# CEED/Laghos

Measured on AMD Instinct MI355X. Metric: Mdofs×steps/s on 3D Sedov -pa (Q3/Q2), higher is better.
Workload: dtype f64; 1 GPU; 3D Sedov -p 1 -m cube01_hex -rs 4 -ok 3 -ot 2 -pa (32^3 elements, E0/2^dim = 0.125); transport=none (one rank), elements=32768, h1_dofs=2738019, l2_dofs=884736, quad_points_per_element=216, rk_stages_executed=1300, ode=RK4, parallelism=elements1x1x1, zones_per_gpu=32x32x32

## Files before the change

include/laghos_hip.h:

```cpp
#ifndef LAGHOS_HIP_H
#define LAGHOS_HIP_H

#ifdef __cplusplus
extern "C" {
#endif

#define LGH_OK 0
#define LGH_ERR_ARG 1
#define LGH_ERR_UNSUPPORTED 2
#define LGH_ERR_HIP 3
#define LGH_ERR_COMM 4

#define LGH_SPACE_H1 0
#define LGH_SPACE_L2 1

typedef struct lgh_ctx lgh_ctx;

typedef struct lgh_config
{
   int dim, NE;
   int D1D, Q1D, L1D;
   int N;
   const int *h1_map;
   const double *B_h1;
// ... 38 lines not shown
int lgh_force_mult(lgh_ctx *ctx, const double *x_l2, double *y_h1);
int lgh_force_mult_transpose(lgh_ctx *ctx, const double *v_h1, double *y_l2);

int lgh_mass_set_essential_tdofs(lgh_ctx *ctx, int comp);
int lgh_mass_eliminate_rhs(lgh_ctx *ctx, double *b);
int lgh_mass_mult(lgh_ctx *ctx, int space, const double *x, double *y);
int lgh_mass_mult_full(lgh_ctx *ctx, int space, const double *x, double *y);

int lgh_cg_solve(lgh_ctx *ctx, int space, const double *b, double *x, double rel_tol,
                 int max_iter, int *iters);
int lgh_l2_mass_solve_local(lgh_ctx *ctx, const double *b, double *x);

int lgh_qupdate(lgh_ctx *ctx, const double *S);
int lgh_qupdate_set_tiny_grad(lgh_ctx *ctx, double tiny_grad);
int lgh_set_fused_forces(lgh_ctx *ctx, int on);
int lgh_qupdate_store_stress(lgh_ctx *ctx, int on);
int lgh_qupdate_stores_stress(lgh_ctx *ctx, int *on);
int lgh_qupdate_form(lgh_ctx *ctx, int *form);
int lgh_reset_quadrature_data(lgh_ctx *ctx);
int lgh_fused_force_mult(lgh_ctx *ctx, double *y_h1);
int lgh_fused_force_mult_transpose(lgh_ctx *ctx, double *y_l2);
int lgh_quadrature_generation(lgh_ctx *ctx, unsigned long *gen, int *f1_valid, int *ftv_valid);
int lgh_get_fused_forces(lgh_ctx *ctx, int *f1, int *ftv);

int lgh_solve_velocity(lgh_ctx *ctx, const double *S, double *dS_dt, const double *one_l2,
                       double *rhs_h1, double *work_B, double rel_tol, int max_iter,
                       int *h1_iters);
int lgh_solve_energy(lgh_ctx *ctx, const double *S, const double *v_h1, double *dS_dt,
                     double *e_rhs, const double *e_source, double rel_tol, int max_iter,
                     int *l2_iters);
// ... 117 lines not shown
```

laghos_amd/_lib.py:

```python
import ctypes
import os

_HERE = os.path.dirname(os.path.abspath(__file__))
LIB_PATH = os.path.join(_HERE, "liblaghos_hip.so")

c_dp = ctypes.c_void_p
c_int_p = ctypes.POINTER(ctypes.c_int)
c_dbl_p = ctypes.POINTER(ctypes.c_double)


class LghConfig(ctypes.Structure):
    _fields_ = [
        ("dim", ctypes.c_int), ("NE", ctypes.c_int),
        ("D1D", ctypes.c_int), ("Q1D", ctypes.c_int), ("L1D", ctypes.c_int),
        ("N", ctypes.c_int),
        ("h1_map", c_int_p),
        ("B_h1", c_dbl_p), ("G_h1", c_dbl_p), ("B_l2", c_dbl_p),
        ("weights", c_dbl_p), ("gamma", c_dbl_p),
        ("ess_count", ctypes.c_int * 3),
        ("ess", c_int_p * 3),
        ("owner", c_dbl_p),
        ("use_viscosity", ctypes.c_int), ("use_vorticity", ctypes.c_int),
        ("cfl", ctypes.c_double),
        ("order_v", ctypes.c_int),
# ... 22 lines not shown
    "lgh_mass_diag": (_P, [_P]),
    "lgh_set_h0": (_I, [_P, _D]),
    "lgh_get_h0": (_I, [_P, c_dbl_p]),
    "lgh_set_dt_est": (_I, [_P, _D]),
    "lgh_get_dt_est": (_I, [_P, c_dbl_p]),
    "lgh_setup_rho0detj0": (_I, [_P, _P, _P, _P, c_dbl_p]),
    "lgh_force_mult": (_I, [_P, _P, _P]),
    "lgh_force_mult_transpose": (_I, [_P, _P, _P]),
    "lgh_mass_set_essential_tdofs": (_I, [_P, _I]),
    "lgh_mass_eliminate_rhs": (_I, [_P, _P]),
    "lgh_mass_mult": (_I, [_P, _I, _P, _P]),
    "lgh_mass_mult_full": (_I, [_P, _I, _P, _P]),
    "lgh_cg_solve": (_I, [_P, _I, _P, _P, _D, _I, c_int_p]),
    "lgh_l2_mass_solve_local": (_I, [_P, _P, _P]),
    "lgh_qupdate": (_I, [_P, _P]),
    "lgh_solve_velocity": (_I, [_P, _P, _P, _P, _P, _P, _D, _I, c_int_p]),
    "lgh_solve_energy": (_I, [_P, _P, _P, _P, _P, _P, _D, _I, c_int_p]),
    "lgh_solve_energy_begin": (_I, [_P, _P, _P, _P, _P, _P, _D, _I]),
    "lgh_tg_source_2d": (_I, [_P, _P, _P]),
    "lgh_set_velocity_source": (_I, [_P, _P]),
    "lgh_solve_energy_end": (_I, [_P, c_int_p]),
    "lgh_vec_set": (_I, [_P, _P, _D, _L]),
    "lgh_vec_copy": (_I, [_P, _P, _P, _L]),
    "lgh_vec_axpby": (_I, [_P, _P, _D, _P, _D, _P, _L]),
    "lgh_vec_axpby_pair": (_I, [_P, _P, _D, _P, _D, _P, _D, _P, _D, _P, _L]),
    "lgh_vec_dot": (_I, [_P, _P, _P, _L, c_dbl_p]),
    "lgh_vec_fingerprint": (_I, [_P, _P, _L, ctypes.c_ulonglong, ctypes.POINTER(ctypes.c_ulonglong)]),
    "lgh_vec_fingerprint_shape": (_I, [_P, _P, _L, ctypes.POINTER(ctypes.c_long)]),
    "lgh_fingerprint_host": (_I, [_P, _L, ctypes.c_ulonglong, ctypes.POINTER(ctypes.c_ulonglong)]),
    "lgh_internal_energy": (_I, [_P, _P, c_dbl_p]),
# ... 98 lines not shown
```

laghos_amd/context.py:

```python
import ctypes

import numpy as np
import torch

from . import _lib
from ._lib import LghConfig, check


def _np_i32(a):
    return np.ascontiguousarray(a, dtype=np.int32)


def _np_f64(a):
    return np.ascontiguousarray(a, dtype=np.float64)


def _ptr(t):
    assert t.is_cuda and t.dtype == torch.float64 and t.is_contiguous()
    return ctypes.c_void_p(t.data_ptr())


def _dbl(a):
    assert isinstance(a, np.ndarray) and a.dtype == np.float64 and a.flags.c_contiguous
    return a.ctypes.data_as(_lib.c_dbl_p)
# ... 205 lines not shown
    def mass_mult(self, space, x, y, full=False):
        fn = self.lib.lgh_mass_mult_full if full else self.lib.lgh_mass_mult
        check(fn(self.h, space, _ptr(x), _ptr(y)))

    def cg_solve(self, space, b, x, rel_tol, max_iter):
        it = ctypes.c_int(0)
        check(self.lib.lgh_cg_solve(self.h, space, _ptr(b), _ptr(x), rel_tol, max_iter, ctypes.byref(it)))
        return it.value

    def l2_mass_solve_local(self, b, x):
        check(self.lib.lgh_l2_mass_solve_local(self.h, _ptr(b), _ptr(x)))

    def qupdate(self, S):
        check(self.lib.lgh_qupdate(self.h, _ptr(S)))

    def qupdate_set_tiny_grad(self, v):
        check(self.lib.lgh_qupdate_set_tiny_grad(self.h, float(v)))

    def table_symmetry(self):
        a, b = ctypes.c_int(-1), ctypes.c_int(-1)
        check(self.lib.lgh_table_symmetry(self.h, ctypes.byref(a), ctypes.byref(b)))
        return a.value, b.value

    def k1_form(self):
        f = ctypes.c_int(-2)
        check(self.lib.lgh_k1_form(self.h, ctypes.byref(f)))
        return {0: "column", 2: "plane", 4: "slab", 5: "kron"}.get(f.value)

    def mesh_order(self):
        o = (ctypes.c_long * 8)()
# ... 273 lines not shown
```

laghos_amd/csrc/lgh_api.hip:

```cpp
#include <cstdarg>
#include <cstdlib>
#include <cmath>
#include <algorithm>
#include <limits>

#include "lgh_common.hpp"

#include <chrono>
#include <dlfcn.h>

namespace lgh
{

static thread_local char g_err[512] = "";
void set_error(const char *fmt, ...)
{
   va_list ap;
   va_start(ap, fmt);
   vsnprintf(g_err, sizeof(g_err), fmt, ap);
   va_end(ap);
}

__global__ void __launch_bounds__(256) vec_set_k(double *y, double a, long n)
{
// ... 489 lines not shown
   LGH_TRY(dev_alloc_zero(&c->Jac0inv_e, (size_t)cfg->NE * dim * dim));
   LGH_TRY(dev_alloc_zero(&c->rho0DetJ0w, nq));
   LGH_TRY(dev_alloc_zero(&c->massD, nq + 2048));
   LGH_TRY(dev_alloc_zero(&c->diagV, (size_t)c->N));
   LGH_TRY(dev_alloc_zero(&c->dinvV, (size_t)c->N));
   LGH_TRY(dev_alloc_zero(&c->dt_est_dev, (size_t)kDtSlotStride * (1 + kDtSlots)));
   {
      const char *env = getenv("LGH_FUSED_FTV");
      if (!(env && env[0] == '0'))
      {
         LGH_TRY(dev_alloc_zero(&c->erhs_q, (size_t)c->L2V));
         LGH_TRY(dev_alloc_zero(&c->v_snap, (size_t)c->H1V));
      }
      LGH_TRY(dev_alloc_zero(&c->dev_flags, (size_t)8));
      c->mass_rank1 = -1;
      env = getenv("LGH_FUSED_F1");
      if (c->dim == 3 && !(env && env[0] == '0')) { LGH_TRY(dev_alloc_zero(&c->force_e_q, nmap * dim + (size_t)dim * c->ND)); }
   }
   const size_t ne_nd = nmap * dim;
   LGH_TRY(dev_alloc_zero(&c->XE, std::max<size_t>(ne_nd, (size_t)c->L2V)));
   LGH_TRY(dev_alloc_zero(&c->YE, ne_nd + (size_t)dim * c->ND));
   const size_t nv = std::max<size_t>((size_t)c->N, (size_t)c->L2V);
   LGH_TRY(dev_alloc_zero(&c->cg_r, nv));
   LGH_TRY(dev_alloc_zero(&c->cg_z, nv));
   LGH_TRY(dev_alloc_zero(&c->cg_d0, nv));
   LGH_TRY(dev_alloc_zero(&c->cg_d1, nv));
   LGH_TRY(dev_alloc_zero(&c->cg_y, nv));
   c->part_stride = (int)std::max<size_t>(std::max<size_t>((size_t)c->NE, (nv + 255) / 256), 2048) + (int)kShards;
   LGH_TRY(dev_alloc_zero(&c->partials, 4 * (size_t)c->part_stride));
   LGH_TRY(dev_alloc_zero(&c->tickets, 4 * (size_t)kTicketSlot));
// ... 269 lines not shown
   if (c->dim == 1) { return cg_1d(c, space, b, x, rel_tol, max_iter, iters, false); }
   return cg_solve(c, space, b, x, rel_tol, max_iter, iters, false);
}

int lgh_l2_mass_solve_local(lgh_ctx *c, const double *b, double *x)
{
   LGH_CHECK_ARG(c && b && x);
   if (c->dim != 1)
   {
      set_error("lgh_l2_mass_solve_local: the zone-local energy solve belongs to the 1D (full-assembly) path; 2D/3D run the energy CG");
      return LGH_ERR_UNSUPPORTED;
   }
   return l2_solve_local_1d(c, b, x);
}

int lgh_qupdate(lgh_ctx *c, const double *S)
{
   LGH_CHECK_ARG(c && S);
   RoctxRange range("QUpdate-UpdateQuadratureData");
   timer_start(c);
   kt_begin(c, LGH_KERNEL_QUPDATE);
   int rc = (c->dim == 1) ? qupdate_1d(c, S) : qupdate(c, S);
   kt_end(c, LGH_KERNEL_QUPDATE);
   timer_stop(c, 3);
   c->timers.c[2] += c->NE;
   return rc;
}

__global__ void __launch_bounds__(256) not_all_ones_k(const double *x, const long n, int *flag)
{
   const long i = (long)blockIdx.x * blockDim.x + threadIdx.x;
   if (i < n && x[i] != 1.0) { *flag = 1; }
}
static bool is_the_one_vector(lgh_ctx *c, const double *one_l2)
{
   if (!one_l2) { return true; }
   int *flag = c->dev_flags + 1;
   if (hipMemsetAsync(flag, 0, sizeof(int), c->stream) != hipSuccess) { return false; }
   hipLaunchKernelGGL(not_all_ones_k, dim3(ceil_div(c->L2V, 256)), dim3(256), 0, c->stream, one_l2, (long)c->L2V, flag);
   int h = 1;
   if (hipMemcpyAsync(&h, flag, sizeof(int), hipMemcpyDeviceToHost, c->stream) != hipSuccess) { return false; }
// ... 163 lines not shown
   if (i < n) { y[i] = x[i]; }
}
__global__ void __launch_bounds__(256) copy_unless_k(double *__restrict__ y, const double *__restrict__ x, const long n, const int *__restrict__ flag)
{
   if (*flag != 0) { return; }
   const long i = (long)blockIdx.x * blockDim.x + threadIdx.x;
   if (i < n) { y[i] = x[i]; }
}
static int energy_rhs(lgh_ctx *c, const double *v_h1, double *e_rhs)
{
   RoctxRange range("SolveEnergy-ForcePA");
   if (c->erhs_q && c->fused_ftv_valid)
   {
      int *flag = c->dev_flags + (c->on_stream2 ? 2 : 0);
      LGH_HIP_CHECK(hipMemsetAsync(flag, 0, sizeof(int), c->stream));
      hipLaunchKernelGGL(vec_differs_k, dim3(grid_for((c->H1V + 1) / 2)), dim3(256), 0, c->stream, v_h1, c->v_snap, (long)c->H1V, flag);
      LGH_HIP_CHECK(hipGetLastError());
      if (c->stress_current)
      {
         const int rc = force_mult_t_L(c, c->stressJinvT, v_h1, e_rhs, flag);
         if (rc) { return rc; }
         hipLaunchKernelGGL(copy_unless_k, dim3(ceil_div(c->L2V, 256)), dim3(256), 0, c->stream, e_rhs, c->erhs_q, (long)c->L2V, flag);
      }
      else
      {
         hipLaunchKernelGGL(erhs_take_or_poison_k, dim3(ceil_div(c->L2V, 256)), dim3(256), 0, c->stream, e_rhs, c->erhs_q, (long)c->L2V, flag, c->dev_flags + 4);
      }
      LGH_HIP_CHECK(hipGetLastError());
      return LGH_OK;
   }
   return lgh_force_mult_transpose(c, v_h1, e_rhs);
// ... 420 lines not shown
```

laghos_amd/csrc/lgh_common.hpp:

```cpp
#pragma once
#include <hip/hip_runtime.h>

#include <cstdint>
#include <cstdio>
#include <cstring>
#include <string>
#include <vector>

#include "../../include/laghos_hip.h"

namespace lgh
{

void set_error(const char *fmt, ...);

#define LGH_HIP_CHECK(expr)                                                              \
   do                                                                                    \
   {                                                                                     \
      hipError_t e_ = (expr);                                                            \
      if (e_ != hipSuccess)                                                              \
      {                                                                                  \
         lgh::set_error("HIP error %s at %s:%d: %s", hipGetErrorName(e_), __FILE__,      \
                        __LINE__, #expr);                                                \
         return LGH_ERR_HIP;                                                             \
// ... 88 lines not shown
   int ess_count[3];
   double *owner;
   int cur_ess;

   double *stressJinvT, *Jac0inv, *rho0DetJ0w, *massD, *diagV, *dinvV;
   double *Jac0inv_soa;
   double *Jac0inv_e;
   int jac0_compact;
   double *massS, *ones_ne;
   double *M1h = nullptr, *M1l = nullptr;
   double *w1d = nullptr;
   int mass_rank1;
   double *dt_est_dev;
   double *erhs_q;
   double *v_snap;
   double *force_e_q;
   int fused_ftv_valid, fused_f1_valid;
   unsigned long qgen;
   int *dev_flags;
   double *ones_l2;
   int stress_store;
   int stress_current;
   int fused_forces_off;
   double *XE;
   double *YE;
   double *cg_r, *cg_z, *cg_d0, *cg_d1, *cg_y;
   double *partials;
   int part_stride;
   unsigned int *tickets;
   lgh::CgScalars *cgs;
// ... 274 lines not shown
struct LockstepWords { const long long *own; const long long *peers; int n_peers, before; };
bool l2_lockstep_possible(lgh_ctx *c);
int cg_l2_begin_lockstep(lgh_ctx *c, const double *b, double *x, double rel_tol, int max_iter);
int l2_lockstep_limit(lgh_ctx *c);
int l2_lockstep_apply(lgh_ctx *c, int it, const LockstepWords &prev, double *den_mirror);
int l2_lockstep_update(lgh_ctx *c, int it, const double *den_src, long long *word_out);
int l2_lockstep_fold(lgh_ctx *c, int it, const LockstepWords &last);
int cg_l2_end_lockstep(lgh_ctx *c, int *iters);
int comm_ranks_before(const lgh_ctx *c);
bool vcg_lockstep_ready(const lgh_ctx *c);
int cg_l2_begin(lgh_ctx *c, const double *b, double *x, double rel_tol, int max_iter);
int cg_l2_end(lgh_ctx *c, int *iters);
void cg_l2_free(lgh_ctx *c);
int cg_solve(lgh_ctx *c, int space, const double *b, double *x, double rel_tol, int max_iter,
             int *iters, bool x_is_zero);
int qupdate(lgh_ctx *c, const double *S);
int setup_rho0detj0(lgh_ctx *c, const double *x0, const double *rho0_l2, const double *rho0_q,
                    double *volume);
int interp_energy(lgh_ctx *c, int which, const double *vec, double *result);
int tg_source_2d(lgh_ctx *c, const double *S, double *out);
int test_eig(lgh_ctx *c, int dim, int n, const double *A, double *lambda, double *vec);
int test_singular(lgh_ctx *c, int dim, int n, const double *A, double *sv);
int test_sqrt(lgh_ctx *c, int n, const double *x, double *y);
int vec_set(lgh_ctx *c, double *y, double a, long n);
int vec_axpby(lgh_ctx *c, double *z, double a, const double *x, double b, const double *y, long n);
int vec_axpby_pair(lgh_ctx *c, double *z1, double a1, const double *x1, double b1, double *z2, double a2, const double *x2, double b2,
                   const double *y, long n);
int vec_neg_inplace(lgh_ctx *c, double *y, long n);
int vec_zero_list(lgh_ctx *c, double *y, const int *list, int n);
int vec_dot(lgh_ctx *c, const double *x, const double *y, const double *w, long n, double *dev_out);
struct HaloNodeAlias { const int *nodes, *sh_node; };
// ... 70 lines not shown
```

laghos_amd/csrc/lgh_qupdate.hip:

```cpp
#include "lgh_qpoint.hpp"
#include "lgh_qrows.hpp"

namespace lgh
{

int qupdate_form(lgh_ctx *c);
int qupdate(lgh_ctx *c, const double *S)
{
   QArgs a = q_base(c);
   a.x = S;
   a.v = S + c->H1V;
   a.e = S + 2 * (size_t)c->H1V;
   a.result = c->dt_est_dev;
   a.Jac0inv_e = (c->jac0_compact == 1) ? c->Jac0inv_e : nullptr;
   const bool keep = !c->stress_store && a.erhs_q && a.force_e && c->v_snap;
   if (keep) { a.stressJinvT = nullptr; }
   const int form = qupdate_form(c);
   const int rc = (form == 1) ? launch_qrows(c, a) : launch_q<QMODE_UPDATE>(c, a);
   c->qgen++;
   c->stress_current = (rc == LGH_OK && !keep) ? 1 : 0;
   c->fused_ftv_valid = (rc == LGH_OK && a.erhs_q && c->v_snap) ? 1 : 0;
   c->fused_f1_valid = (rc == LGH_OK && a.force_e) ? 1 : 0;
   if (c->fused_ftv_valid)
   {
      LGH_HIP_CHECK(hipMemcpyAsync(c->v_snap, S + c->H1V, sizeof(double) * (size_t)c->H1V, hipMemcpyDeviceToDevice, c->stream));
   }
   return rc;
}

int qupdate_form(lgh_ctx *c)
{
   const char *fenv = getenv("LGH_Q_FORM");
   return (qrows_available(c) && !(fenv && fenv[0] == '0')) ? 1 : 0;
}

int interp_energy(lgh_ctx *c, int which, const double *vec, double *result)
{
   QArgs a = q_base(c);
   a.result = c->scal;
   int rc;
// ... 130 lines not shown
```

laghos_amd/csrc/lgh_vcg.hip:

```cpp
#include "lgh_vcg.hpp"

namespace lgh
{
typedef unsigned v4u_ __attribute__((ext_vector_type(4)));


template <int D, int Q, int NEB>
__global__ void __launch_bounds__(Q *Q *NEB, (Q >= 8) ? 1 : 2)
vcg_apply_3d(const VcgArgs a, const int nbatch)
{
   constexpr int NQ = Q * Q * Q, ND = D * D * D;
   constexpr int SX = (ND > D * Q * Q) ? ND : D * Q * Q;
   constexpr int SA = D * D * Q;
   constexpr int SAE = (SA > D * Q * D) ? SA : D * Q * D;
   constexpr int OFF_A = kVC * SX, OFF_IN = OFF_A + kVC * SAE;
   constexpr int PER = OFF_IN + kVC * ND + 1;
   constexpr int NT = Q * Q * NEB;
   constexpr int GPT = (NEB * ND + NT - 1) / NT;
   __shared__ double smem[NEB * PER];
   __shared__ double red[48];

   if (a.s->all_done) { return; }
   const int tid = threadIdx.x;
   const int tx = tid % Q, ty = (tid / Q) % Q, eb = tid / (Q * Q);
// ... 986 lines not shown
         VcgScalars *s = a.s;
         int all = 1;
         vcg_reset_scalars(a, s);
         for (int c = 0; c < kVC; c++)
         {
            s->rz[c] = s->rz_prev[c] = total[c];
            s->iters[c] = 0;
            s->r0[c] = fmax(total[c] * s->rel_tol2, 0.0);
            s->done[c] = (total[c] < 0.0 || total[c] <= s->r0[c]) ? 1 : 0;
            all = all && s->done[c];
         }
         s->first = 1;
         s->all_done = all;
      }
   }
}
__global__ void __launch_bounds__(256)
vcg_ellf_k(const int *__restrict__ ell, unsigned *__restrict__ ellf, const size_t n_have, const size_t n_all, const int ND, const int NE)
{
   const size_t i = (size_t)blockIdx.x * blockDim.x + threadIdx.x;
   if (i >= n_all) { return; }
   const int p = (i < n_have) ? ell[i] : -1;
   const int e = p / ND;
   ellf[i] = 8u * (unsigned)(p < 0 ? kVC * ND * NE : kVC * ND * e + (p - e * ND));
}
__global__ void __launch_bounds__(256)
vcg_mapb_k(const int *__restrict__ map, unsigned *__restrict__ mapb, const size_t n)
{
   const size_t i = (size_t)blockIdx.x * blockDim.x + threadIdx.x;
   if (i < n) { mapb[i] = 8u * (unsigned)map[i]; }
// ... 431 lines not shown
            }
            all = all && s->done[k];
         }
         if (!a.multi) { s->all_done = all; }
         if (a.pack_rz)
         {
            for (int k = 0; k < a.hp.n_nbr; k++)
            {
               for (int e = 0; e < kVC; e++) { a.hp.sbuf[(size_t)a.hp.base[k] + e] = s->rz[e]; }
            }
         }
      }
   }
}
__global__ void __launch_bounds__(256)
vcg_xfix_k(const VcgArgs a)
{
   const int n = blockIdx.x * blockDim.x + threadIdx.x;
   if (n >= a.N) { return; }
   for (int k = 0; k < kVC; k++)
   {
      if ((a.s->nupd[k] & 1) == 0) { continue; }
      const size_t i = (size_t)k * a.N + n;
      a.x[i] = fma(a.s->alpha_last[k], a.d[i], a.x[i]);
   }
}

__global__ void __launch_bounds__(256)
vcg_xout_k(const VcgArgs a, double *__restrict__ X)
{
   const int n = blockIdx.x * blockDim.x + threadIdx.x;
   if (n >= a.N) { return; }
   const int nc = a.ncaller[n];
   for (int k = 0; k < kVC; k++)
   {
      const size_t i = (size_t)k * a.N + n;
      double xv = a.x[i];
      if (a.s->nupd[k] & 1) { xv = fma(a.s->alpha_last[k], a.d[i], xv); }
      X[(size_t)k * a.N + nc] = xv;
   }
}

__global__ void __launch_bounds__(256)
vcg_gather_k(const VcgArgs a)
{
   const int n = blockIdx.x * blockDim.x + threadIdx.x;
   if (n >= a.N) { return; }
   for (int c = 0; c < kVC; c++)
   {
      if (a.s->done[c]) { continue; }
      const double *yc = a.YE + (size_t)c * a.ye_stride;
      double s = 0.0;
// ... 179 lines not shown
   if (c->multi) { comm_shared_nodes(c, &hmask, &sh_node, &n_shared); }
   hipLaunchKernelGGL(vcg_essbits_k, dim3((unsigned)((c->N + 255) / 256)), dim3(256), 0, nullptr, c->essmask[0], c->essmask[1],
                      c->essmask[2], hmask, c->multi ? c->owner : nullptr, *out, c->N);
   LGH_HIP_CHECK(hipGetLastError());
   return LGH_OK;
}


struct VcgAux
{
   double *ye = nullptr;
   unsigned *ellz = nullptr;
   uint8_t *essbits = nullptr;
   int *nstart = nullptr;
   unsigned *ellf = nullptr;
   unsigned *mapb = nullptr;
   int map_xrows = 0;
   long long *limbs = nullptr;
   long long *rzl = nullptr;
   int grid2 = 0;
   int rz_words_all = -1;
   int rz_words_key = -1;
   int ls_all = 0;
   int ls_ready = 0;
   unsigned *settab = nullptr;
   int *ellm = nullptr;
   int degm = 0;
   unsigned *ellzm = nullptr;
   int *nstartm = nullptr;
   const MeshOrder *ord = nullptr;
// ... 18 lines not shown
   return LGH_OK;
}
void vcg_free(lgh_ctx *c)
{
   VcgAux *x = (VcgAux *)c->vcg_aux;
   if (!x) { return; }
   (void)hipFree(x->settab);
   (void)hipFree(x->ellm);
   (void)hipFree(x->ellzm);
   (void)hipFree(x->nstartm);
   (void)hipFree(x->ye);
   (void)hipFree(x->ellz);
   (void)hipFree(x->essbits);
   (void)hipFree(x->nstart);
   (void)hipFree(x->ellf);
   (void)hipFree(x->mapb);
   (void)hipFree(x->limbs);
   (void)hipFree(x->rzl);
   (void)hipFree(x->o_map);
   (void)hipFree(x->o_ell);
   (void)hipFree(x->o_ellc);
   for (int k = 0; k < kVC; k++) { (void)hipFree(x->o_ess[k]); }
   (void)hipFree(x->o_dinv);
   (void)hipFree(x->o_Se);
   (void)hipFree(x->o_massD);
   (void)hipFree(x->o_x);
   (void)hipFree(x->o_owner);
   (void)hipFree(x->o_hmask);
   (void)hipFree(x->o_nodes);
   (void)hipFree(x->o_shnode);
// ... 276 lines not shown
         {
            uint8_t *tmp = nullptr;
            LGH_HIP_CHECK(hipMalloc((void **)&tmp, (size_t)c->N));
            LGH_HIP_CHECK(hipStreamSynchronize(nullptr));
            rc = order_gather_bytes(c, x->essbits, tmp);
            if (rc) { (void)hipFree(tmp); return rc; }
            LGH_HIP_CHECK(hipStreamSynchronize(c->stream));
            (void)hipFree(x->essbits);
            x->essbits = tmp;
         }
         rc = partition_nodes_by_cost(c, x->grid2, &x->nstart, x->ord ? &x->o_valence : nullptr);
         if (rc) { return rc; }
         if ((size_t)kVC * (c->NE + 1) * c->ND * 8 < 0xffffffffull)
         {
            const size_t ell_n = (size_t)8 * c->N;
            LGH_HIP_CHECK(hipMalloc((void **)&x->ellf, ell_n * sizeof(unsigned)));
            hipLaunchKernelGGL(vcg_ellf_k, dim3((unsigned)((ell_n + 255) / 256)), dim3(256), 0, nullptr, x->o_ellc ? x->o_ellc : c->t_ell, x->ellf,
                               (size_t)c->t_deg * c->N, ell_n, c->ND, c->NE);
            LGH_HIP_CHECK(hipGetLastError());
         }
      }
      if (vcg_k1_form(c) == 4)
      {
         const size_t nm = (size_t)c->NE * c->ND;
         LGH_HIP_CHECK(hipMalloc((void **)&x->mapb, nm * sizeof(unsigned)));
         hipLaunchKernelGGL(vcg_mapb_k, dim3((unsigned)((nm + 255) / 256)), dim3(256), 0, nullptr, v_map, x->mapb, nm);
         LGH_HIP_CHECK(hipGetLastError());
         int *flag = (int *)c->scal, h = 1;
         LGH_HIP_CHECK(hipMemset(flag, 0, sizeof(int)));
         hipLaunchKernelGGL(vcg_map_xrows_k, dim3((unsigned)((nm / c->D1D + 255) / 256)), dim3(256), 0, nullptr, v_map, nm / c->D1D, c->D1D, flag);
         LGH_HIP_CHECK(hipMemcpy(&h, flag, sizeof(int), hipMemcpyDeviceToHost));
         x->map_xrows = (h == 0) ? 1 : 0;
         LGH_HIP_CHECK(hipMalloc((void **)&x->limbs, (2 * kLimbWords + 8 * 16 + 32 * 4096) * sizeof(long long)));
// ... 241 lines not shown
int vcg_solve(lgh_ctx *c, double *B, double *X, double rel_tol, int max_iter, int iters[3], const double *force_E)
{
   if (!vcg_supported(c)) { return LGH_ERR_UNSUPPORTED; }
   VcgPlan plan;
   int rc = vcg_prepare(c, B, X, rel_tol, plan, true);
   if (rc) { return rc; }
   VcgArgs &a = plan.a;
   VcgAux *aux = plan.aux;
   const bool k2p = plan.k2p;
   const bool multi = c->multi != 0;
   const size_t N = (size_t)c->N;
   VcgScalars *ds = (VcgScalars *)c->vcg_s;
   const int nb = ceil_div((long)N, 256);
   const HaloNodeAlias *alias = (aux->ord && aux->o_alias.nodes) ? &aux->o_alias : nullptr;

   a.partials = c->vcg_partials;
   a.ticket = c->vcg_tickets;
   if (force_E)
   {
      if (multi || c->t_deg > 8) { set_error("vcg_solve: fused init is single-rank, degree <= 8"); return LGH_ERR_ARG; }
      if (aux->ellf && aux->essbits)
      {
         hipLaunchKernelGGL(vcg_init_force_z_k, dim3(nb), dim3(256), 0, c->stream, a, force_E, 8u * (unsigned)c->ND, aux->ellf, B);
      }
      else { hipLaunchKernelGGL(vcg_init_force_k<8>, dim3(nb), dim3(256), 0, c->stream, a, force_E, c->ND, B, aux->o_ellc ? aux->o_ellc : c->t_ell, c->t_deg); }
   }
   else
   {
      if (aux->ord) { LGH_HIP_CHECK(hipMemsetAsync(a.x, 0, kVC * N * sizeof(double), c->stream)); }
      hipLaunchKernelGGL(vcg_init_k, dim3(nb), dim3(256), 0, c->stream, a);
   }
   LGH_HIP_CHECK(hipGetLastError());
   if (multi)
   {
      rc = allreduce_dev(c, ds->rz, kVC, 0);
      if (rc) { return rc; }
// ... 25 lines not shown
   if (ls_side) { rc = hand_over(c->ev_fork, false); if (rc) { return rc; } }
   int chunk = c->vcg_last > 0 ? c->vcg_last : 8;
   bool first_look = true;
   while (true)
   {
      if (!first_look || max_iter <= 0)
      {
         VcgScalars *hs_dev = (VcgScalars *)(c->host_pinned_dev + 32);
         unsigned long long *tok_dev = (unsigned long long *)(c->host_pinned_dev + 80);
         volatile unsigned long long *tok = (volatile unsigned long long *)(c->host_pinned + 80);
         const unsigned long long token = ++c->look_token;
         bool copied = false;
         if (!energy_polled) { rc = energy_overlap_poll(c); energy_polled = true; if (rc) { return rc; } }
         if (multi && !a.rzl && it > 0) { hipLaunchKernelGGL(vcg_update_finish_k, dim3(1), dim3(1), 0, c->stream, ds, it, hs_dev, tok_dev, token); copied = true; }
         if (a.rzl && it > 0) { hipLaunchKernelGGL(vcg_rz_finish_k, dim3(1), dim3(1), 0, c->stream, ds, a.rzl, it, a.rzl_peers, a.n_rz_peers, hs_dev, tok_dev, token); copied = true; }
         if (copied)
         {
            rc = host_wait_token(c, tok, token);
            if (rc) { return rc; }
         }
         else
         {
            LGH_HIP_CHECK(hipMemcpyAsync(hs, ds, sizeof(VcgScalars), hipMemcpyDeviceToHost, c->stream));
            LGH_HIP_CHECK(hipStreamSynchronize(c->stream));
         }
         if (hs->all_done || it >= max_iter) { break; }
         chunk = (++looks <= 2) ? 2 : std::min(64, 2 * chunk);
      }
      first_look = false;
      const int upto = std::min(max_iter, it + chunk);
// ... 77 lines not shown
               {
                  rc = side([&] { return l2_lockstep_fold(c, it, ls_words(it)); });
                  if (rc) { return rc; }
               }
            }
            else if (multi)
            {
               rc = allreduce_dev(c, ds->rz, kVC, 0, a.pack_rz != 0 && mixed && k2p);
               if (rc) { return rc; }
            }
         }
         LGH_HIP_CHECK(hipGetLastError());
      }
   }
   if (ls_side) { rc = hand_over(c->ev_join, true); if (rc) { return rc; } }
   if (aux->ord)
   {
      hipLaunchKernelGGL(vcg_xout_k, dim3(nb), dim3(256), 0, c->stream, a, X);
      LGH_HIP_CHECK(hipGetLastError());
   }
   else if (k2p && ((hs->nupd[0] | hs->nupd[1] | hs->nupd[2]) & 1))
   {
      hipLaunchKernelGGL(vcg_xfix_k, dim3(nb), dim3(256), 0, c->stream, a);
      LGH_HIP_CHECK(hipGetLastError());
   }
   if (trace_dev)
   {
      std::vector<unsigned long long> h(kTraceRec * 4096);
      (void)hipMemcpy(h.data(), trace_dev, h.size() * 8, hipMemcpyDeviceToHost);
      FILE *f = fopen(trace_path, "w");
      if (f)
      {
         for (int i = 0; i < 4096; i++)
         {
            if (h[(size_t)kTraceRec * i] == 0) { continue; }
            fprintf(f, "%d", i);
            for (int k = 0; k < kTraceRec; k++) { fprintf(f, " %llu", h[(size_t)kTraceRec * i + k]); }
            fprintf(f, "\n");
// ... 423 lines not shown
```

laghos_amd/host/laghos_solver.cpp:

```cpp
#include "laghos_solver.hpp"

#include <cmath>
#include <cstdlib>
#include <cstring>
#include <iomanip>
#include <iostream>
#include <limits>

namespace laghos
{
namespace hydrodynamics
{

void AbortWithLghError(const char *where)
{
   std::fprintf(stderr, "%s failed: %s\n", where, lgh_last_error());
   std::abort();
}

LagrangianHydroOperator::LagrangianHydroOperator(const Discretization &d, const std::vector<double> &S0,
                                                 const std::vector<double> &rho0_l2,
                                                 const std::vector<double> &gamma,
                                                 const std::vector<double> &rho0_q, double cfl,
                                                 double cgt, int cgiter, int device, const char *nccl_id)
// ... 82 lines not shown
   {
      std::vector<double> acc((size_t)H1Vsize, 0.0);
      for (long i = H1Vsize / dim; i < 2 * (H1Vsize / dim); i++) { acc[i] = -1.0; }
      accel_src.FromHost(acc);
      LGH_VERIFY(lgh_set_velocity_source(ctx, accel_src.Read()));
   }
   B.SetSize(d.N);
   LGH_VERIFY(lgh_sync(ctx));
}

LagrangianHydroOperator::~LagrangianHydroOperator() { lgh_destroy(ctx); }

void LagrangianHydroOperator::Mult(const Vector &S, Vector &dS_dt) const
{
   UpdateMesh(S);
   LGH_VERIFY(lgh_vec_copy(ctx, dS_dt.Write(), S.Read() + H1Vsize, H1Vsize));
   UpdateQuadratureData(S);
   if (source_type == 1) { LGH_VERIFY(lgh_tg_source_2d(ctx, S.Read(), e_source.Write())); }
   LGH_VERIFY(lgh_solve_energy_begin(ctx, S.Read(), S.Read() + H1Vsize, dS_dt.Write(), e_rhs.Write(),
                                     source_type == 1 ? e_source.Read() : nullptr, cg_rel_tol, cg_max_iter));
   SolveVelocity(S, dS_dt);
   int it = 0;
   LGH_VERIFY(lgh_solve_energy_end(ctx, &it));
   qdata_is_current = false;
}

void LagrangianHydroOperator::SolveVelocity(const Vector &S, Vector &dS_dt) const
{
   UpdateQuadratureData(S);
   int it = 0;
   LGH_VERIFY(lgh_solve_velocity(ctx, S.Read(), dS_dt.Write(), nullptr, rhs.Write(), B.Write(),
                                 cg_rel_tol, cg_max_iter, &it));
}

void LagrangianHydroOperator::SolveEnergy(const Vector &S, const Vector &v, Vector &dS_dt) const
{
   UpdateQuadratureData(S);
   int it = 0;
   if (source_type == 1) { LGH_VERIFY(lgh_tg_source_2d(ctx, S.Read(), e_source.Write())); }
   LGH_VERIFY(lgh_solve_energy(ctx, S.Read(), v.Read(), dS_dt.Write(), e_rhs.Write(),
                               source_type == 1 ? e_source.Read() : nullptr,
                               cg_rel_tol, cg_max_iter, &it));
}

void LagrangianHydroOperator::UpdateQuadratureData(const Vector &S) const
{
   unsigned long gen = 0;
   int f1 = 0, ftv = 0;
   LGH_VERIFY(lgh_quadrature_generation(ctx, &gen, &f1, &ftv));
   if (qdata_is_current && gen == qdata_gen) { return; }
   qdata_is_current = true;
   qupdate->UpdateQuadratureData(S, *qdata);
   LGH_VERIFY(lgh_quadrature_generation(ctx, &gen, &f1, &ftv));
   qdata_gen = gen;
}

double LagrangianHydroOperator::GetTimeStepEstimate(const Vector &S) const
{
   UpdateMesh(S);
   UpdateQuadratureData(S);
   double dt = qdata->GetDtEst();
   if (disc.part.nranks > 1) { LGH_VERIFY(lgh_allreduce(ctx, &dt, 1)); }
   return dt;
}

void LagrangianHydroOperator::ResetTimeStepEstimate() const
{
   qdata->SetDtEst(std::numeric_limits<double>::infinity());
}
// ... 351 lines not shown
```

laghos_amd/host/laghos_solver.hpp:

```cpp
#pragma once
#include <memory>

#include "fem.hpp"
#include "laghos_assembly.hpp"

namespace laghos
{
namespace hydrodynamics
{

struct TimingData
{
   double sw_cgH1 = 0, sw_cgL2 = 0, sw_force = 0, sw_qdata = 0;
   long L2dof = 0, H1iter = 0, L2iter = 0, quad_tstep = 0;
};

class QUpdate
{
   lgh_ctx *ctx;

public:
   explicit QUpdate(lgh_ctx *c) : ctx(c) {}
   void UpdateQuadratureData(const Vector &S, QuadratureData &) { LGH_VERIFY(lgh_qupdate(ctx, S.Read())); }
};

class LagrangianHydroOperator
{
protected:
   const Discretization &disc;
   lgh_ctx *ctx;
   const int dim, NE;
   const int H1Vsize, L2Vsize;
   const long H1GTVSize, L2GTVSize;
   const double cg_rel_tol;
   const int cg_max_iter;
   std::unique_ptr<QuadratureData> qdata;
   mutable bool qdata_is_current;
   mutable unsigned long qdata_gen = 0;
// ... 9 lines not shown

public:
   LagrangianHydroOperator(const Discretization &disc, const std::vector<double> &S0,
                           const std::vector<double> &rho0_l2, const std::vector<double> &gamma,
                           const std::vector<double> &rho0_q, double cfl, double cgt, int cgiter,
                           int device, const char *nccl_id);
   ~LagrangianHydroOperator();

   int Size() const { return 2 * H1Vsize + L2Vsize; }
   int H1VSize() const { return H1Vsize; }
   int L2VSize() const { return L2Vsize; }
   void Mult(const Vector &S, Vector &dS_dt) const;
   void SolveVelocity(const Vector &S, Vector &dS_dt) const;
   void SolveEnergy(const Vector &S, const Vector &v, Vector &dS_dt) const;
   void UpdateMesh(const Vector &) const {}
   void UpdateQuadratureData(const Vector &S) const;
   double GetTimeStepEstimate(const Vector &S) const;
   void ResetTimeStepEstimate() const;
   void ResetQuadratureData() const { qdata_is_current = false; LGH_VERIFY(lgh_reset_quadrature_data(ctx)); }
   double InternalEnergy(const Vector &S) const;
   double KineticEnergy(const Vector &S) const;
   double ENorm(const Vector &S) const;
   void ComputeDensity(const Vector &S, Vector &rho) const;
   double SedovDensityError(const Vector &S, const Vector &rho, const double par[21], double t,
                            const double origin[3], int err_order) const;
   void SampleFields(const Vector &S, const Vector &rho, int R, Vector &out) const;
   long SamplePoints(int R) const;
   void Diagnostics(const Vector &S, double out[LGH_DIAG_COUNT]) const;
   void Profile(const Vector &S, const lgh_profile_spec &spec, double *rows, long *n_excluded) const;
   void SedovEval(const double par[21], double t, const std::vector<double> &r, std::vector<double> &rho, std::vector<double> &v,
                  std::vector<double> &p) const;
// ... 103 lines not shown
```

Measured before the change: 1596 Mdofs*steps/s.

## Reuse dS_dt velocity copy as snapshot and fold CG x-zeroing into finish kernels

In the default stage-fast mode, the velocity copy into dS_dt doubles as the quadrature-update velocity snapshot, so the separate v_snap copy is no longer needed. The velocity CG fused force-init kernel gets a variant with a per-row skip of the upper table half that can leave x unzeroed, and the x fix-up/output kernels now overwrite x for components with fewer than two updates. The x-finish kernel is launched speculatively inside the iteration loop, gated on all_done. The aim is to remove one device copy and one zero-fill per stage, at the cost of extra kernel launches per iteration and more complex correctness invariants.

Result: no change. 1608 Mdofs*steps/s (median of 6 runs) (+0.7%).

```diff
diff --git a/include/laghos_hip.h b/include/laghos_hip.h
--- a/include/laghos_hip.h
+++ b/include/laghos_hip.h
@@ -76,6 +76,8 @@
 int lgh_qupdate(lgh_ctx *ctx, const double *S);
 int lgh_qupdate_set_tiny_grad(lgh_ctx *ctx, double tiny_grad);
 int lgh_set_fused_forces(lgh_ctx *ctx, int on);
+int lgh_qupdate_snapshot(lgh_ctx *ctx, const double *S, double *v_copy);
+int lgh_stage_fast(lgh_ctx *ctx, int *on);
 int lgh_qupdate_store_stress(lgh_ctx *ctx, int on);
 int lgh_qupdate_stores_stress(lgh_ctx *ctx, int *on);
 int lgh_qupdate_form(lgh_ctx *ctx, int *form);
diff --git a/laghos_amd/_lib.py b/laghos_amd/_lib.py
--- a/laghos_amd/_lib.py
+++ b/laghos_amd/_lib.py
@@ -60,6 +60,8 @@
     "lgh_cg_solve": (_I, [_P, _I, _P, _P, _D, _I, c_int_p]),
     "lgh_l2_mass_solve_local": (_I, [_P, _P, _P]),
     "lgh_qupdate": (_I, [_P, _P]),
+    "lgh_qupdate_snapshot": (_I, [_P, _P, _P]),
+    "lgh_stage_fast": (_I, [_P, c_int_p]),
     "lgh_solve_velocity": (_I, [_P, _P, _P, _P, _P, _P, _D, _I, c_int_p]),
     "lgh_solve_energy": (_I, [_P, _P, _P, _P, _P, _P, _D, _I, c_int_p]),
     "lgh_solve_energy_begin": (_I, [_P, _P, _P, _P, _P, _P, _D, _I]),
diff --git a/laghos_amd/context.py b/laghos_amd/context.py
--- a/laghos_amd/context.py
+++ b/laghos_amd/context.py
@@ -243,6 +243,14 @@
     def qupdate(self, S):
         check(self.lib.lgh_qupdate(self.h, _ptr(S)))
 
+    def qupdate_snapshot(self, S, v_copy):
+        check(self.lib.lgh_qupdate_snapshot(self.h, _ptr(S), _ptr(v_copy)))
+
+    def stage_fast(self):
+        on = ctypes.c_int(-1)
+        check(self.lib.lgh_stage_fast(self.h, ctypes.byref(on)))
+        return bool(on.value)
+
     def qupdate_set_tiny_grad(self, v):
         check(self.lib.lgh_qupdate_set_tiny_grad(self.h, float(v)))
 
diff --git a/laghos_amd/csrc/lgh_api.hip b/laghos_amd/csrc/lgh_api.hip
--- a/laghos_amd/csrc/lgh_api.hip
+++ b/laghos_amd/csrc/lgh_api.hip
@@ -527,6 +527,8 @@
       }
       LGH_TRY(dev_alloc_zero(&c->dev_flags, (size_t)8));
       c->mass_rank1 = -1;
+      env = getenv("LGH_STAGE_FAST");
+      c->stage_fast = (env && env[0] == '0') ? 0 : 1;
       env = getenv("LGH_FUSED_F1");
       if (c->dim == 3 && !(env && env[0] == '0')) { LGH_TRY(dev_alloc_zero(&c->force_e_q, nmap * dim + (size_t)dim * c->ND)); }
    }
@@ -826,17 +828,34 @@
    return l2_solve_local_1d(c, b, x);
 }
 
-int lgh_qupdate(lgh_ctx *c, const double *S)
-{
-   LGH_CHECK_ARG(c && S);
+static int qupdate_entry(lgh_ctx *c, const double *S, double *v_copy)
+{
    RoctxRange range("QUpdate-UpdateQuadratureData");
    timer_start(c);
    kt_begin(c, LGH_KERNEL_QUPDATE);
-   int rc = (c->dim == 1) ? qupdate_1d(c, S) : qupdate(c, S);
+   int rc = (c->dim == 1) ? qupdate_1d(c, S) : qupdate(c, S, v_copy);
    kt_end(c, LGH_KERNEL_QUPDATE);
    timer_stop(c, 3);
    c->timers.c[2] += c->NE;
    return rc;
+}
+int lgh_qupdate(lgh_ctx *c, const double *S)
+{
+   LGH_CHECK_ARG(c && S);
+   return qupdate_entry(c, S, nullptr);
+}
+static bool energy_overlap_ok(const lgh_ctx *c);
+int lgh_stage_fast(lgh_ctx *c, int *on)
+{
+   LGH_CHECK_ARG(c && on);
+   *on = (c->stage_fast && c->dim != 1 && energy_overlap_ok(c)) ? 1 : 0;
+   return LGH_OK;
+}
+int lgh_qupdate_snapshot(lgh_ctx *c, const double *S, double *v_copy)
+{
+   LGH_CHECK_ARG(c && S && v_copy);
+   if (c->dim == 1) { set_error("lgh_qupdate_snapshot: 2D/3D only (the 1D path keeps no velocity copy)"); return LGH_ERR_UNSUPPORTED; }
+   return qupdate_entry(c, S, v_copy);
 }
 
 __global__ void __launch_bounds__(256) not_all_ones_k(const double *x, const long n, int *flag)
@@ -1030,7 +1049,7 @@
    {
       int *flag = c->dev_flags + (c->on_stream2 ? 2 : 0);
       LGH_HIP_CHECK(hipMemsetAsync(flag, 0, sizeof(int), c->stream));
-      hipLaunchKernelGGL(vec_differs_k, dim3(grid_for((c->H1V + 1) / 2)), dim3(256), 0, c->stream, v_h1, c->v_snap, (long)c->H1V, flag);
+      hipLaunchKernelGGL(vec_differs_k, dim3(grid_for((c->H1V + 1) / 2)), dim3(256), 0, c->stream, v_h1, c->v_snap_cur ? c->v_snap_cur : c->v_snap, (long)c->H1V, flag);
       LGH_HIP_CHECK(hipGetLastError());
       if (c->stress_current)
       {
diff --git a/laghos_amd/csrc/lgh_common.hpp b/laghos_amd/csrc/lgh_common.hpp
--- a/laghos_amd/csrc/lgh_common.hpp
+++ b/laghos_amd/csrc/lgh_common.hpp
@@ -126,6 +126,8 @@
    double *dt_est_dev;
    double *erhs_q;
    double *v_snap;
+   const double *v_snap_cur = nullptr;
+   int stage_fast = 1;
    double *force_e_q;
    int fused_ftv_valid, fused_f1_valid;
    unsigned long qgen;
@@ -430,7 +432,7 @@
 void cg_l2_free(lgh_ctx *c);
 int cg_solve(lgh_ctx *c, int space, const double *b, double *x, double rel_tol, int max_iter,
              int *iters, bool x_is_zero);
-int qupdate(lgh_ctx *c, const double *S);
+int qupdate(lgh_ctx *c, const double *S, double *v_copy = nullptr);
 int setup_rho0detj0(lgh_ctx *c, const double *x0, const double *rho0_l2, const double *rho0_q,
                     double *volume);
 int interp_energy(lgh_ctx *c, int which, const double *vec, double *result);
diff --git a/laghos_amd/csrc/lgh_qupdate.hip b/laghos_amd/csrc/lgh_qupdate.hip
--- a/laghos_amd/csrc/lgh_qupdate.hip
+++ b/laghos_amd/csrc/lgh_qupdate.hip
@@ -5,7 +5,7 @@
 {
 
 int qupdate_form(lgh_ctx *c);
-int qupdate(lgh_ctx *c, const double *S)
+int qupdate(lgh_ctx *c, const double *S, double *v_copy)
 {
    QArgs a = q_base(c);
    a.x = S;
@@ -21,9 +21,10 @@
    c->stress_current = (rc == LGH_OK && !keep) ? 1 : 0;
    c->fused_ftv_valid = (rc == LGH_OK && a.erhs_q && c->v_snap) ? 1 : 0;
    c->fused_f1_valid = (rc == LGH_OK && a.force_e) ? 1 : 0;
-   if (c->fused_ftv_valid)
+   c->v_snap_cur = v_copy ? v_copy : c->v_snap;
+   if (c->fused_ftv_valid || v_copy)
    {
-      LGH_HIP_CHECK(hipMemcpyAsync(c->v_snap, S + c->H1V, sizeof(double) * (size_t)c->H1V, hipMemcpyDeviceToDevice, c->stream));
+      LGH_HIP_CHECK(hipMemcpyAsync(v_copy ? v_copy : c->v_snap, S + c->H1V, sizeof(double) * (size_t)c->H1V, hipMemcpyDeviceToDevice, c->stream));
    }
    return rc;
 }
diff --git a/laghos_amd/csrc/lgh_vcg.hip b/laghos_amd/csrc/lgh_vcg.hip
--- a/laghos_amd/csrc/lgh_vcg.hip
+++ b/laghos_amd/csrc/lgh_vcg.hip
@@ -1024,6 +1024,98 @@
          s->all_done = all;
       }
    }
+}
+__global__ void __launch_bounds__(256)
+vcg_init_force_z2_k(const VcgArgs a, const double *__restrict__ FE, const unsigned compb_fe, const unsigned *__restrict__ ellfz,
+                    double *__restrict__ bout, const int zero_x)
+{
+   vcg_reset_accumulators(a);
+   __shared__ double red[48];
+   const int n = xcd_swizzle(blockIdx.x, gridDim.x) * blockDim.x + threadIdx.x;
+   const bool ok = n < a.N;
+   const unsigned nn = (unsigned)(ok ? n : a.N - 1);
+   const v4u_ q0 = *(const v4u_ *)((const char *)ellfz + 16u * nn);
+   const double di = vcg_ld(a.dinv, 8u * nn);
+   const unsigned es = a.essbits[nn];
+   const unsigned zoff = 8u * (unsigned)kVC * (unsigned)(a.ye_stride - kYePad);
+   const bool hi = __any(q0[3] != zoff);
+   double sum[kVC];
+   {
+      double fe[kVC][4];
+#pragma unroll
+      for (int j = 0; j < 4; j++)
+      {
+         if (j == 0 || __any(q0[j] != zoff))
+         {
+#pragma unroll
+            for (int c = 0; c < kVC; c++) { fe[c][j] = vcg_ld(FE, q0[j] + (unsigned)c * compb_fe); }
+         }
+         else
+         {
+#pragma unroll
+            for (int c = 0; c < kVC; c++) { fe[c][j] = 0.0; }
+         }
+      }
+#pragma unroll
+      for (int c = 0; c < kVC; c++) { sum[c] = (((0.0 + fe[c][0]) + fe[c][1]) + fe[c][2]) + fe[c][3]; }
+   }
+   if (hi)
+   {
+      const v4u_ q1 = *(const v4u_ *)((const char *)ellfz + (size_t)16 * (size_t)a.N + 16u * nn);
+#pragma unroll
+      for (int c = 0; c < kVC; c++)
+      {
+         const unsigned cb = (unsigned)c * compb_fe;
+         const double f4 = vcg_ld(FE, q1[0] + cb), f5 = vcg_ld(FE, q1[1] + cb), f6 = vcg_ld(FE, q1[2] + cb), f7 = vcg_ld(FE, q1[3] + cb);
+         sum[c] = (((sum[c] + f4) + f5) + f6) + f7;
+      }
+   }
+   double part[kVC];
+#pragma unroll
+   for (int c = 0; c < kVC; c++)
+   {
+      double bv = -sum[c];
+      if ((es >> c) & 1u) { bv = 0.0; }
+      part[c] = ok ? __dmul_rn(bv, di) * bv : 0.0;
+      if (ok)
+      {
+         const size_t i = (size_t)c * a.N + n;
+         bout[(size_t)c * a.N + (a.ncaller ? a.ncaller[n] : n)] = bv;
+         a.r[i] = bv;
+         if (zero_x) { a.x[i] = 0.0; }
+      }
+   }
+   double bp[kVC], total[kVC];
+   block_sum3(part[0], part[1], part[2], red, bp);
+   if (grid_sum3_last_block(bp, a.partials, a.stride, a.ticket, red, total))
+   {
+      if (threadIdx.x == 0)
+      {
+         VcgScalars *s = a.s;
+         int all = 1;
+         vcg_reset_scalars(a, s);
+         for (int c = 0; c < kVC; c++)
+         {
+            s->rz[c] = s->rz_prev[c] = total[c];
+            s->iters[c] = 0;
+            s->r0[c] = fmax(total[c] * s->rel_tol2, 0.0);
+            s->done[c] = (total[c] < 0.0 || total[c] <= s->r0[c]) ? 1 : 0;
+            all = all && s->done[c];
+         }
+         s->first = 1;
+         s->all_done = all;
+      }
+   }
+}
+__global__ void __launch_bounds__(256)
+vcg_ellfz_k(const int *__restrict__ ell, unsigned *__restrict__ ellfz, const size_t n_have, const size_t n_all, const int ND, const int NE)
+{
+   const size_t i = (size_t)blockIdx.x * blockDim.x + threadIdx.x;
+   if (i >= n_all) { return; }
+   const int p = (i < n_have) ? ell[i] : -1;
+   const int e = p / ND;
+   const size_t N = n_all / 8, j = i / N, n = i - j * N;
+   ellfz[(j < 4 ? 0 : 4 * N) + 4 * n + (j & 3)] = 8u * (unsigned)(p < 0 ? kVC * ND * NE : kVC * ND * e + (p - e * ND));
 }
 __global__ void __launch_bounds__(256)
 vcg_ellf_k(const int *__restrict__ ell, unsigned *__restrict__ ellf, const size_t n_have, const size_t n_all, const int ND, const int NE)
@@ -1485,28 +1577,32 @@
    }
 }
 __global__ void __launch_bounds__(256)
-vcg_xfix_k(const VcgArgs a)
-{
+vcg_xfix_k(const VcgArgs a, const int mode)
+{
+   if (mode == 1 && !a.s->all_done) { return; }
    const int n = blockIdx.x * blockDim.x + threadIdx.x;
    if (n >= a.N) { return; }
    for (int k = 0; k < kVC; k++)
    {
-      if ((a.s->nupd[k] & 1) == 0) { continue; }
+      const int nu = a.s->nupd[k];
       const size_t i = (size_t)k * a.N + n;
+      if (mode != 0 && nu < 2) { a.x[i] = (nu == 0) ? 0.0 : fma(a.s->alpha_last[k], a.d[i], 0.0); continue; }
+      if ((nu & 1) == 0) { continue; }
       a.x[i] = fma(a.s->alpha_last[k], a.d[i], a.x[i]);
    }
 }
 
 __global__ void __launch_bounds__(256)
-vcg_xout_k(const VcgArgs a, double *__restrict__ X)
-{
+vcg_xout_k(const VcgArgs a, double *__restrict__ X, const int mode)
+{
+   if (mode == 1 && !a.s->all_done) { return; }
    const int n = blockIdx.x * blockDim.x + threadIdx.x;
    if (n >= a.N) { return; }
    const int nc = a.ncaller[n];
    for (int k = 0; k < kVC; k++)
    {
       const size_t i = (size_t)k * a.N + n;
-      double xv = a.x[i];
+      double xv = (mode != 0 && a.s->nupd[k] < 2) ? 0.0 : a.x[i];
       if (a.s->nupd[k] & 1) { xv = fma(a.s->alpha_last[k], a.d[i], xv); }
       X[(size_t)k * a.N + nc] = xv;
    }
@@ -1716,6 +1812,7 @@
    uint8_t *essbits = nullptr;
    int *nstart = nullptr;
    unsigned *ellf = nullptr;
+   unsigned *ellfz = nullptr;
    unsigned *mapb = nullptr;
    int map_xrows = 0;
    long long *limbs = nullptr;
@@ -1764,6 +1861,7 @@
    (void)hipFree(x->essbits);
    (void)hipFree(x->nstart);
    (void)hipFree(x->ellf);
+   (void)hipFree(x->ellfz);
    (void)hipFree(x->mapb);
    (void)hipFree(x->limbs);
    (void)hipFree(x->rzl);
@@ -2070,9 +2168,10 @@
          if ((size_t)kVC * (c->NE + 1) * c->ND * 8 < 0xffffffffull)
          {
             const size_t ell_n = (size_t)8 * c->N;
-            LGH_HIP_CHECK(hipMalloc((void **)&x->ellf, ell_n * sizeof(unsigned)));
-            hipLaunchKernelGGL(vcg_ellf_k, dim3((unsigned)((ell_n + 255) / 256)), dim3(256), 0, nullptr, x->o_ellc ? x->o_ellc : c->t_ell, x->ellf,
-                               (size_t)c->t_deg * c->N, ell_n, c->ND, c->NE);
+            unsigned **tab = c->stage_fast ? &x->ellfz : &x->ellf;
+            LGH_HIP_CHECK(hipMalloc((void **)tab, ell_n * sizeof(unsigned)));
+            hipLaunchKernelGGL(c->stage_fast ? vcg_ellfz_k : vcg_ellf_k, dim3((unsigned)((ell_n + 255) / 256)), dim3(256), 0, nullptr,
+                               x->o_ellc ? x->o_ellc : c->t_ell, *tab, (size_t)c->t_deg * c->N, ell_n, c->ND, c->NE);
             LGH_HIP_CHECK(hipGetLastError());
          }
       }
@@ -2344,12 +2443,18 @@
    const int nb = ceil_div((long)N, 256);
    const HaloNodeAlias *alias = (aux->ord && aux->o_alias.nodes) ? &aux->o_alias : nullptr;
 
+   const bool x_set = c->stage_fast && k2p && !multi;
+   bool x_finished = false;
    a.partials = c->vcg_partials;
    a.ticket = c->vcg_tickets;
    if (force_E)
    {
       if (multi || c->t_deg > 8) { set_error("vcg_solve: fused init is single-rank, degree <= 8"); return LGH_ERR_ARG; }
-      if (aux->ellf && aux->essbits)
+      if (aux->ellfz && aux->essbits)
+      {
+         hipLaunchKernelGGL(vcg_init_force_z2_k, dim3(nb), dim3(256), 0, c->stream, a, force_E, 8u * (unsigned)c->ND, aux->ellfz, B, x_set ? 0 : 1);
+      }
+      else if (aux->ellf && aux->essbits)
       {
          hipLaunchKernelGGL(vcg_init_force_z_k, dim3(nb), dim3(256), 0, c->stream, a, force_E, 8u * (unsigned)c->ND, aux->ellf, B);
       }
@@ -2405,6 +2510,14 @@
          if (!energy_polled) { rc = energy_overlap_poll(c); energy_polled = true; if (rc) { return rc; } }
          if (multi && !a.rzl && it > 0) { hipLaunchKernelGGL(vcg_update_finish_k, dim3(1), dim3(1), 0, c->stream, ds, it, hs_dev, tok_dev, token); copied = true; }
          if (a.rzl && it > 0) { hipLaunchKernelGGL(vcg_rz_finish_k, dim3(1), dim3(1), 0, c->stream, ds, a.rzl, it, a.rzl_peers, a.n_rz_peers, hs_dev, tok_dev, token); copied = true; }
+         if (x_set && a.rzl && it > 0)
+         {
+            const int mode = (it >= max_iter) ? 2 : 1;
+            if (aux->ord) { hipLaunchKernelGGL(vcg_xout_k, dim3(nb), dim3(256), 0, c->stream, a, X, mode); }
+            else { hipLaunchKernelGGL(vcg_xfix_k, dim3(nb), dim3(256), 0, c->stream, a, mode); }
+            LGH_HIP_CHECK(hipGetLastError());
+            x_finished = true;
+         }
          if (copied)
          {
             rc = host_wait_token(c, tok, token);
@@ -2512,14 +2625,15 @@
       }
    }
    if (ls_side) { rc = hand_over(c->ev_join, true); if (rc) { return rc; } }
-   if (aux->ord)
-   {
-      hipLaunchKernelGGL(vcg_xout_k, dim3(nb), dim3(256), 0, c->stream, a, X);
+   if (x_finished) {  }
+   else if (aux->ord)
+   {
+      hipLaunchKernelGGL(vcg_xout_k, dim3(nb), dim3(256), 0, c->stream, a, X, x_set ? 2 : 0);
       LGH_HIP_CHECK(hipGetLastError());
    }
-   else if (k2p && ((hs->nupd[0] | hs->nupd[1] | hs->nupd[2]) & 1))
-   {
-      hipLaunchKernelGGL(vcg_xfix_k, dim3(nb), dim3(256), 0, c->stream, a);
+   else if (x_set || (k2p && ((hs->nupd[0] | hs->nupd[1] | hs->nupd[2]) & 1)))
+   {
+      hipLaunchKernelGGL(vcg_xfix_k, dim3(nb), dim3(256), 0, c->stream, a, x_set ? 2 : 0);
       LGH_HIP_CHECK(hipGetLastError());
    }
    if (trace_dev)
diff --git a/laghos_amd/host/laghos_solver.cpp b/laghos_amd/host/laghos_solver.cpp
--- a/laghos_amd/host/laghos_solver.cpp
+++ b/laghos_amd/host/laghos_solver.cpp
@@ -120,8 +120,14 @@
 void LagrangianHydroOperator::Mult(const Vector &S, Vector &dS_dt) const
 {
    UpdateMesh(S);
-   LGH_VERIFY(lgh_vec_copy(ctx, dS_dt.Write(), S.Read() + H1Vsize, H1Vsize));
-   UpdateQuadratureData(S);
+   int fast = 0;
+   LGH_VERIFY(lgh_stage_fast(ctx, &fast));
+   if (!fast)
+   {
+      LGH_VERIFY(lgh_vec_copy(ctx, dS_dt.Write(), S.Read() + H1Vsize, H1Vsize));
+      UpdateQuadratureData(S);
+   }
+   else if (!UpdateQuadratureData(S, dS_dt.Write())) { LGH_VERIFY(lgh_vec_copy(ctx, dS_dt.Write(), S.Read() + H1Vsize, H1Vsize)); }
    if (source_type == 1) { LGH_VERIFY(lgh_tg_source_2d(ctx, S.Read(), e_source.Write())); }
    LGH_VERIFY(lgh_solve_energy_begin(ctx, S.Read(), S.Read() + H1Vsize, dS_dt.Write(), e_rhs.Write(),
                                      source_type == 1 ? e_source.Read() : nullptr, cg_rel_tol, cg_max_iter));
@@ -149,16 +155,18 @@
                                cg_rel_tol, cg_max_iter, &it));
 }
 
-void LagrangianHydroOperator::UpdateQuadratureData(const Vector &S) const
+bool LagrangianHydroOperator::UpdateQuadratureData(const Vector &S, double *v_copy) const
 {
    unsigned long gen = 0;
    int f1 = 0, ftv = 0;
    LGH_VERIFY(lgh_quadrature_generation(ctx, &gen, &f1, &ftv));
-   if (qdata_is_current && gen == qdata_gen) { return; }
+   if (qdata_is_current && gen == qdata_gen) { return false; }
    qdata_is_current = true;
-   qupdate->UpdateQuadratureData(S, *qdata);
+   if (v_copy) { qupdate->UpdateQuadratureData(S, *qdata, v_copy); }
+   else { qupdate->UpdateQuadratureData(S, *qdata); }
    LGH_VERIFY(lgh_quadrature_generation(ctx, &gen, &f1, &ftv));
    qdata_gen = gen;
+   return v_copy != nullptr;
 }
 
 double LagrangianHydroOperator::GetTimeStepEstimate(const Vector &S) const
diff --git a/laghos_amd/host/laghos_solver.hpp b/laghos_amd/host/laghos_solver.hpp
--- a/laghos_amd/host/laghos_solver.hpp
+++ b/laghos_amd/host/laghos_solver.hpp
@@ -22,6 +22,7 @@
 public:
    explicit QUpdate(lgh_ctx *c) : ctx(c) {}
    void UpdateQuadratureData(const Vector &S, QuadratureData &) { LGH_VERIFY(lgh_qupdate(ctx, S.Read())); }
+   void UpdateQuadratureData(const Vector &S, QuadratureData &, double *v_copy) { LGH_VERIFY(lgh_qupdate_snapshot(ctx, S.Read(), v_copy)); }
 };
 
 class LagrangianHydroOperator
@@ -61,7 +62,7 @@
    void SolveVelocity(const Vector &S, Vector &dS_dt) const;
    void SolveEnergy(const Vector &S, const Vector &v, Vector &dS_dt) const;
    void UpdateMesh(const Vector &) const {}
-   void UpdateQuadratureData(const Vector &S) const;
+   bool UpdateQuadratureData(const Vector &S, double *v_copy = nullptr) const;
    double GetTimeStepEstimate(const Vector &S) const;
    void ResetTimeStepEstimate() const;
    void ResetQuadratureData() const { qdata_is_current = false; LGH_VERIFY(lgh_reset_quadrature_data(ctx)); }
```
